# huangjh-pub/di-fusion

Hardware: AMD Instinct MI355X
Metric: frames/s integrate+decode+mesh, 640x480 synthetic stream (higher is better)
Workload: dtype f32

## Files before the change

di_fusion_amd/csrc/kernels_extract.hip.h:

```cpp
#pragma once

__device__ __forceinline__ void mark_confident_nbhd(const Geo& g, int lin, float ignore_th, const int64_t* __restrict__ indexer,
                                                    const float* __restrict__ obs, const GridMarks& marks) {
    const uint32_t* bits = marks.bits;
    int ix, iy, iz;
    unlinearize(g, lin, ix, iy, iz);
    int cand[7];
    cand[0] = lin;
    cand[1] = linearize(g, clampi(ix - 1, 0, g.nx - 1), iy, iz);
    cand[2] = linearize(g, clampi(ix + 1, 0, g.nx - 1), iy, iz);
    cand[3] = linearize(g, ix, clampi(iy - 1, 0, g.ny - 1), iz);
    cand[4] = linearize(g, ix, clampi(iy + 1, 0, g.ny - 1), iz);
    cand[5] = linearize(g, ix, iy, clampi(iz - 1, 0, g.nz - 1));
    cand[6] = linearize(g, ix, iy, clampi(iz + 1, 0, g.nz - 1));
    int64_t slot[7];
#pragma unroll
    for (int c = 0; c < 7; ++c) slot[c] = indexer[cand[c]];
    float w[7];
#pragma unroll
    for (int c = 0; c < 7; ++c) w[c] = slot[c] >= 0 ? obs[slot[c]] : ignore_th;
    uint32_t word[7];
#pragma unroll
    for (int c = 0; c < 7; ++c) word[c] = (w[c] > ignore_th) ? bits[cand[c] >> 5] : 0xFFFFFFFFu;
    uint32_t prev[7];
#pragma unroll
    for (int c = 0; c < 7; ++c) {
        const uint32_t b = 1u << (cand[c] & 31);
        prev[c] = (word[c] & b) ? 0xFFFFFFFFu : atomicOr(marks.bits + (cand[c] >> 5), b);
    }
#pragma unroll
    for (int c = 0; c < 7; ++c)
        if (!(prev[c] & (1u << (cand[c] & 31)))) atomicAdd(marks.tot + (cand[c] >> 5) / marks.per_words, 1);
}

__global__ void __launch_bounds__(DIF_BLOCK) k_mark_halo_dirty(Geo g, float ignore_th, uint8_t* __restrict__ dirty, const int64_t* __restrict__ pos,
                                                             const int64_t* __restrict__ indexer, const float* __restrict__ obs,
                                                             GridMarks bits, const int* __restrict__ n_ptr, int64_t own_lo,
                                                             int64_t own_hi) {
    const int n = *n_ptr;
    for (int s = blockIdx.x * blockDim.x + threadIdx.x; s < n; s += gridDim.x * blockDim.x) {
        if (!dirty[s]) continue;
        const int64_t p = pos[s];
        if (p >= own_lo && p < own_hi) continue;
        dirty[s] = 0;
        mark_confident_nbhd(g, (int)p, ignore_th, indexer, obs, bits);
    }
}

struct DirtySet {
    uint8_t* dirty;
    const int64_t* pos;
    int64_t* valid_blocks;
    int* counters;
    int no_cache;
    int64_t max_voxels;
    Geo g;
    float ignore_th;
    const int64_t* indexer;
    const float* obs;
    GridMarks bits;
    int64_t own_lin_lo, own_lin_hi;
    bool tiled;
    __device__ __forceinline__ bool owned(int s) const {
        if (!tiled) return true;
        const int64_t p = pos[s];
        return p >= own_lin_lo && p < own_lin_hi;
    }
};

struct DirtyFunctor {
    DirtySet a;
    __device__ int count(int s) const { return ((a.no_cache || a.dirty[s]) && a.owned(s)) ? 1 : 0; }
    __device__ void emit(int s, int offset) const {
        a.dirty[s] = 0;
        if (offset >= a.max_voxels) return;
        const int lin = (int)a.pos[s];
        a.valid_blocks[offset] = lin;
        mark_confident_nbhd(a.g, lin, a.ignore_th, a.indexer, a.obs, a.bits);
    }
    __device__ void finish(int total) const {
        if (total > a.max_voxels) { total = (int)a.max_voxels; a.counters[DIF_C_OVERFLOW] = 2; }
        a.counters[DIF_C_K] = total;
        a.counters[DIF_C_DEFERRED] = 0;
    }
};

__device__ __forceinline__ void dirty_scan_body(const DirtySet& a, const int* __restrict__ n_ptr, const int* __restrict__ block_tot,
                                                uint32_t* __restrict__ fused_word, int seq) {
    __shared__ int smem[8];
    if (fused_word && blockIdx.x == 0 && threadIdx.x == 0) __hip_atomic_store(fused_word, (uint32_t)seq, __ATOMIC_RELAXED, __HIP_MEMORY_SCOPE_AGENT);
    const int s = (int)blockIdx.x * DIF_BLOCK + (int)threadIdx.x;
    const bool flag = a.dirty[s] != 0;
    if (!__syncthreads_or((int)flag) && blockIdx.x != 0) return;
    int before = 0, all = 0;
    const int n_blk = (int)gridDim.x;
    for (int b = (int)threadIdx.x; b < n_blk; b += DIF_BLOCK) {
        const int t = block_tot[b];
        all += t;
        if (b < (int)blockIdx.x) before += t;
    }
    const GridMarks& marks = a.bits;
    int lin = 0, cand[7];
    uint32_t word[7];
#pragma unroll
    for (int c = 0; c < 7; ++c) { cand[c] = 0; word[c] = 0xFFFFFFFFu; }
    if (flag && (lin = (int)a.pos[s]) >= 0) {
        int ix, iy, iz;
        unlinearize(a.g, lin, ix, iy, iz);
        cand[0] = lin;
        cand[1] = linearize(a.g, clampi(ix - 1, 0, a.g.nx - 1), iy, iz);
        cand[2] = linearize(a.g, clampi(ix + 1, 0, a.g.nx - 1), iy, iz);
        cand[3] = linearize(a.g, ix, clampi(iy - 1, 0, a.g.ny - 1), iz);
        cand[4] = linearize(a.g, ix, clampi(iy + 1, 0, a.g.ny - 1), iz);
        cand[5] = linearize(a.g, ix, iy, clampi(iz - 1, 0, a.g.nz - 1));
        cand[6] = linearize(a.g, ix, iy, clampi(iz + 1, 0, a.g.nz - 1));
        int64_t slot[7];
#pragma unroll
        for (int c = 0; c < 7; ++c) slot[c] = a.indexer[cand[c]];
        float w[7];
#pragma unroll
        for (int c = 0; c < 7; ++c) w[c] = slot[c] >= 0 ? a.obs[slot[c]] : a.ignore_th;
#pragma unroll
        for (int c = 0; c < 7; ++c) word[c] = (w[c] > a.ignore_th) ? marks.bits[cand[c] >> 5] : 0xFFFFFFFFu;
    }
    const int n = *n_ptr;
    const bool mine = flag && s < n;
    int offset = block_sum(before, smem);
    const int total = block_sum(all, smem);
    {
        const int64_t need = min((int64_t)7 * total, (int64_t)n);
        if (need > a.max_voxels) {
            if (blockIdx.x == 0 && threadIdx.x == 0) { a.counters[DIF_C_K] = 0; a.counters[DIF_C_DEFERRED] = (int)need; }
            return;
        }
    }
    int chunk_total;
    const int ex = block_excl_scan(mine ? 1 : 0, smem, chunk_total);
    if (mine) {
        a.dirty[s] = 0;
        if (offset + ex < a.max_voxels) {
            a.valid_blocks[offset + ex] = lin;
            uint32_t prev[7];
#pragma unroll
            for (int c = 0; c < 7; ++c) {
                const uint32_t b = 1u << (cand[c] & 31);
                prev[c] = (word[c] & b) ? 0xFFFFFFFFu : atomicOr(marks.bits + (cand[c] >> 5), b);
            }
#pragma unroll
            for (int c = 0; c < 7; ++c)
                if (!(prev[c] & (1u << (cand[c] & 31)))) atomicAdd(marks.tot + (cand[c] >> 5) / marks.per_words, 1);
        }
    }
    if (blockIdx.x == 0 && threadIdx.x == 0) {
        int t = total;
        if (t > a.max_voxels) { t = (int)a.max_voxels; a.counters[DIF_C_OVERFLOW] = 2; }
        a.counters[DIF_C_K] = t;
        a.counters[DIF_C_DEFERRED] = 0;
    }
}

__global__ void __launch_bounds__(DIF_BLOCK) k_dirty_scan(DirtySet a, const int* __restrict__ n_ptr, const int* __restrict__ block_tot, uint32_t* __restrict__ fused_word, int seq) {
    dirty_scan_body(a, n_ptr, block_tot, fused_word, seq);
}
struct DirtyScanArgs { DirtySet a; const int* n_ptr; const int* block_tot; };
__global__ void __launch_bounds__(DIF_BLOCK) k_dirty_scan_batch(Batch<DirtyScanArgs> b) {
    const DirtyScanArgs& a = b.s[blockIdx.y];
    dirty_scan_body(a.a, a.n_ptr, a.block_tot, nullptr, 0);
}
__global__ void k_publish_word(uint32_t* __restrict__ word, uint32_t value) {
    if (threadIdx.x == 0) __hip_atomic_store(word, value, __ATOMIC_RELAXED, __HIP_MEMORY_SCOPE_AGENT);
}

struct OccFunctor {
    uint32_t* bits;
    const int64_t* indexer;
    int32_t* occ_slot;
    int32_t* vbm;
    int* counters;
    int64_t max_voxels;
    __device__ int count(int w) const { return __popc(bits[w]); }
    __device__ void emit(int w, int offset) const {
        uint32_t word = bits[w];
        bits[w] = 0u;
        while (word) {
            int b = __ffs((int)word) - 1;
            word &= word - 1;
            int slot = (int)indexer[w * 32 + b];
            if (offset < max_voxels) {
                occ_slot[offset] = slot;
                vbm[slot] = offset;
            }
            ++offset;
        }
    }
    __device__ void finish(int total) const {
        if (total > max_voxels) { total = (int)max_voxels; counters[DIF_C_OVERFLOW] = 3; }
        counters[DIF_C_B] = total;
        counters[DIF_C_VH] = 0;
        counters[DIF_C_WORK] = 0;
    }
};

struct Lattice {
    int res;
    float vsize, a;
    __device__ __forceinline__ float coord(int i) const { return ((float)i * vsize + a) - 0.5f; }
};

struct DecodeArgs {
    int mode;
    const int* n_ptr;
    int64_t n_static;
    Lattice lat;
    const int32_t* occ_slot;
    const float* latent;
    const int32_t* list;
    const float* rows;
    const float* xyz;
    const int64_t* indexer;
    Geo geo;
    float* out_sdf;
    float* out_std;
    float sign;
    float* out_grad;
    const float* wbwd;
    float grad_scale;
    const float* fold_table;
    const float* obs;
    float ignore_th;
    float pose[12];
    int* zero_word;
};

__device__ __forceinline__ float pose_row(const float* T, int j, float x, float y, float z) {
    return __fadd_rn(__fadd_rn(__fadd_rn(__fmul_rn(x, T[4 * j]), __fmul_rn(y, T[4 * j + 1])), __fmul_rn(z, T[4 * j + 2])), T[4 * j + 3]);
}

struct DecodeRow { bool live; int64_t out_idx; float px, py, pz; bool bad; };
template <bool DENSE = false>
__device__ __forceinline__ DecodeRow decode_row_input(const DecodeArgs& A, int64_t tile, int col, int half, int res3, int tiles_per_voxel, int64_t n_rows,
                                                      f16v& xin) {
    DecodeRow R{false, 0, 0.f, 0.f, 0.f, false};
    const float* lat_row = nullptr;
    const float* row32 = nullptr;
    if (!DENSE && A.mode == 0) {
        const int64_t b = tile / tiles_per_voxel;
        const int s = (int)(tile - b * tiles_per_voxel) * 32 + col;
        R.live = s < res3;
        if (R.live) {
            const int r = A.lat.res;
            R.px = A.lat.coord(s / (r * r)); R.py = A.lat.coord((s / r) % r); R.pz = A.lat.coord(s % r);
            lat_row = A.latent + (int64_t)A.occ_slot[b] * L;
            R.out_idx = b * res3 + s;
        }
    } else if (!DENSE && A.mode == 1) {
        const int64_t row = tile * 32 + col;
        R.live = row < n_rows;
        if (R.live) {
            const int e = A.list[row];
            const int b = e / res3, s = e - b * res3, r = A.lat.res;
            R.px = A.lat.coord(s / (r * r)); R.py = A.lat.coord((s / r) % r); R.pz = A.lat.coord(s % r);
            lat_row = A.latent + (int64_t)A.occ_slot[b] * L;
            R.out_idx = e;
        }
    } else if (!DENSE && A.mode == 2) {
        const int64_t row = tile * 32 + col;
        R.live = row < n_rows;
        if (R.live) { row32 = A.rows + row * 32; R.out_idx = row; }
    } else if (DENSE) {
        const int64_t row = tile * 32 + col;
        if (row < n_rows) {
            const float x = A.xyz[row * 3 + 0], y = A.xyz[row * 3 + 1], z = A.xyz[row * 3 + 2];
            float xn, yn, zn; int ix, iy, iz;
            bool ok = voxel_of(A.geo, pose_row(A.pose, 0, x, y, z), pose_row(A.pose, 1, x, y, z), pose_row(A.pose, 2, x, y, z), xn, yn, zn, ix, iy, iz);
            int64_t slot = -1;
            if (ok) {
                slot = A.indexer[linearize(A.geo, ix, iy, iz)];
                ok = slot >= 0 && A.obs[slot] > A.ignore_th;
            }
            R.live = ok;
            R.out_idx = row;
            if (ok) {
                R.px = (xn - (float)ix) - 0.5f; R.py = (yn - (float)iy) - 0.5f; R.pz = (zn - (float)iz) - 0.5f;
                lat_row = A.latent + slot * L;
            } else if (half == 1) A.out_std[row] = 0.0f;
        }
    } else {
        const int64_t row = tile * 32 + col;
        R.live = row < n_rows;
        if (R.live) {
            const int64_t p = A.list[row];
            float xn, yn, zn; int ix, iy, iz;
            voxel_of(A.geo, A.xyz[p * 3 + 0], A.xyz[p * 3 + 1], A.xyz[p * 3 + 2], xn, yn, zn, ix, iy, iz);
            R.px = (xn - (float)ix) - 0.5f; R.py = (yn - (float)iy) - 0.5f; R.pz = (zn - (float)iz) - 0.5f;
            lat_row = A.latent + A.indexer[linearize(A.geo, ix, iy, iz)] * L;
            R.out_idx = row;
        }
    }
#pragma unroll
    for (int t = 0; t < 16; ++t) {
        const int k = 2 * t + half;
        float v = 0.0f;
        if (R.live) {
            if (row32) v = row32[k];
            else if (k < L) v = lat_row[k];
            else v = (k == L) ? R.px : ((k == L + 1) ? R.py : R.pz);
        }
        xin[t] = v;
    }
    if constexpr (!DENSE) {
        if (A.mode == 2) {
            unsigned nf = 0;
#pragma unroll
            for (int t = 0; t < 16; ++t) nf |= ((__float_as_uint(xin[t]) & 0x7f800000u) == 0x7f800000u) ? 1u : 0u;
            nf |= (unsigned)__shfl_xor((int)nf, 32);
            R.bad = nf != 0;
        }
    }
    return R;
}

template <bool GRAD, bool DENSE = false>
__global__ void __launch_bounds__(GRAD ? 256 : 512, GRAD ? 1 : 2) k_decode(DecodeArgs A, const float* __restrict__ wblob) {
    extern __shared__ __attribute__((aligned(16))) float lds[];
    if (DENSE && A.zero_word && blockIdx.x == 0 && threadIdx.x == 0) *A.zero_word = 0;
    stage_weights(lds, wblob, DEC_LDS_FLOATS);
    const __amdgpu_buffer_rsrc_t wfwd = make_rsrc(wblob, DEC_FLOATS);
    const __amdgpu_buffer_rsrc_t wbwd = make_rsrc(GRAD ? A.wbwd : wblob, GRAD ? DECB_FLOATS : DEC_FLOATS);
    const int lane = lane_id(), half = lane >> 5, col = lane & 31;
    const int wave = (int)((threadIdx.x >> 6) * gridDim.x + blockIdx.x);
    const int nwaves = (int)(gridDim.x * (blockDim.x >> 6));
    const int res3 = A.lat.res * A.lat.res * A.lat.res;
    const int tiles_per_voxel = (res3 + 31) / 32;
    int64_t n_rows, n_tiles;
    if (A.mode == 0) {
        n_rows = (int64_t)(*A.n_ptr) * res3;
        n_tiles = (int64_t)(*A.n_ptr) * tiles_per_voxel;
    } else {
        n_rows = A.n_ptr ? (int64_t)(*A.n_ptr) : A.n_static;
        n_tiles = (n_rows + 31) / 32;
    }
    for (int64_t tile = wave; tile < n_tiles; tile += nwaves) {
        f16v xin;
        const DecodeRow R = decode_row_input<DENSE>(A, tile, col, half, res3, tiles_per_voxel, n_rows, xin);
        const bool live = R.live;
        const int64_t out_idx = R.out_idx;
        const float px = R.px, py = R.py, pz = R.pz;
        float sdf, sd;
        if (!GRAD && A.mode == 1 && A.fold_table) {
            const int b = live ? A.list[tile * 32 + col] / res3 : 0;
            decoder_tile_folded(lds, wfwd, FoldInitGlobal{A.fold_table + (int64_t)b * 256}, px, py, pz, lane, sdf, sd);
        } else if (GRAD) {
            float gx, gy, gz;
            decoder_tile_grad(lds, wfwd, wbwd, xin, lane, sdf, sd, gx, gy, gz);
            if (live && half == 1) {
                const float gs = R.bad ? __builtin_nanf("") : A.grad_scale;
                A.out_grad[out_idx * 3 + 0] = gx * gs;
                A.out_grad[out_idx * 3 + 1] = gy * gs;
                A.out_grad[out_idx * 3 + 2] = gz * gs;
            }
        } else {
            decoder_tile(lds, wfwd, xin, lane, sdf, sd);
        }
        if (live) {
            if (half == 0) A.out_sdf[out_idx] = R.bad ? __builtin_nanf("") : A.sign * sdf;
            else A.out_std[out_idx] = R.bad ? __builtin_nanf("") : sd;
        }
    }
}

template <bool DENSE = false>
__global__ void __launch_bounds__(512, 1) k_decode_x6(DecodeArgs A, const float* __restrict__ wblob, const float* __restrict__ wu) {
    extern __shared__ __attribute__((aligned(16))) float lds[];
    if (DENSE && A.zero_word && blockIdx.x == 0 && threadIdx.x == 0) *A.zero_word = 0;
    stage_weights(lds, wblob, X6_LDS_BYTES / 4);
    const __amdgpu_buffer_rsrc_t wfwd = make_rsrc(wblob, X6_BYTES / 4);
    const __amdgpu_buffer_rsrc_t wun = make_rsrc(wu, X6U_BYTES / 4);
    const int lane = lane_id(), half = lane >> 5, col = lane & 31;
    const int wave = (int)((threadIdx.x >> 6) * gridDim.x + blockIdx.x);
    const int nwaves = (int)(gridDim.x * (blockDim.x >> 6));
    const int res3 = A.lat.res * A.lat.res * A.lat.res;
    const int tiles_per_voxel = (res3 + 31) / 32;
    int64_t n_rows, n_tiles;
    if (A.mode == 0) {
        n_rows = (int64_t)(*A.n_ptr) * res3;
        n_tiles = (int64_t)(*A.n_ptr) * tiles_per_voxel;
    } else {
        n_rows = A.n_ptr ? (int64_t)(*A.n_ptr) : A.n_static;
        n_tiles = (n_rows + 31) / 32;
    }
    for (int64_t tile = wave; tile < n_tiles; tile += nwaves) {
        f16v xin;
        const DecodeRow R = decode_row_input<DENSE>(A, tile, col, half, res3, tiles_per_voxel, n_rows, xin);
        const bool live = R.live;
        const int64_t out_idx = R.out_idx;
        float sdf, sd;
        decoder_tile_x6(lds, wfwd, wun, xin, lane, sdf, sd);
        if (live) {
            if (half == 0) A.out_sdf[out_idx] = R.bad ? __builtin_nanf("") : A.sign * sdf;
            else A.out_std[out_idx] = R.bad ? __builtin_nanf("") : sd;
        }
    }
}

#ifndef GRAD_X6_THREADS
#define GRAD_X6_THREADS 256
#endif
template <int PF, bool DENSE = false>
__global__ void __launch_bounds__(GRAD_X6_THREADS, 1) k_decode_grad_x6(DecodeArgs A, const float* __restrict__ wblob, const float* __restrict__ wu,
                                                          const float* __restrict__ wb) {
    extern __shared__ __attribute__((aligned(16))) float lds[];
    if (DENSE && A.zero_word && blockIdx.x == 0 && threadIdx.x == 0) *A.zero_word = 0;
    stage_weights(lds, wblob, X6_LDS_BYTES / 4);
    const __amdgpu_buffer_rsrc_t wfwd = make_rsrc(wblob, X6_BYTES / 4);
    const __amdgpu_buffer_rsrc_t wun = make_rsrc(wu, X6U_BYTES / 4);
    const __amdgpu_buffer_rsrc_t wbw = make_rsrc(wb, X6B_BYTES / 4);
    const int lane = lane_id(), half = lane >> 5, col = lane & 31;
    const int wave = (int)((threadIdx.x >> 6) * gridDim.x + blockIdx.x);
    const int nwaves = (int)(gridDim.x * (blockDim.x >> 6));
    const int res3 = A.lat.res * A.lat.res * A.lat.res;
    const int64_t n_rows = A.n_ptr ? (int64_t)(*A.n_ptr) : A.n_static;
    const int64_t n_tiles = (n_rows + 31) / 32;
    for (int64_t tile = wave; tile < n_tiles; tile += nwaves) {
        f16v xin;
        const DecodeRow R = decode_row_input<DENSE>(A, tile, col, half, res3, 1, n_rows, xin);
        float sdf, sd, gx, gy, gz;
        decoder_tile_grad_x6<PF>(lds, wfwd, wun, wbw, xin, lane, sdf, sd, gx, gy, gz);
        if (R.live) {
            if (half == 0) A.out_sdf[R.out_idx] = R.bad ? __builtin_nanf("") : A.sign * sdf;
            else {
                const float gs = R.bad ? __builtin_nanf("") : A.grad_scale;
                A.out_std[R.out_idx] = R.bad ? __builtin_nanf("") : sd;
                A.out_grad[R.out_idx * 3 + 0] = gx * gs;
                A.out_grad[R.out_idx * 3 + 1] = gy * gs;
                A.out_grad[R.out_idx * 3 + 2] = gz * gs;
            }
        }
    }
}

template <int NS>
__device__ __forceinline__ void decode_refine_x6_body(const BatchN<DecodeArgs, NS>& B, int S, const float* __restrict__ wblob) {
    extern __shared__ __attribute__((aligned(16))) float lds[];
    const int lane = lane_id(), half = lane >> 5, col = lane & 31;
    const int wave = __builtin_amdgcn_readfirstlane((int)((threadIdx.x >> 6) * gridDim.x + blockIdx.x));
    const int nwaves = (int)(gridDim.x * (blockDim.x >> 6));
    const Lattice lat = B.s[0].lat;
    const float sign = B.s[0].sign;
    const int res3 = lat.res * lat.res * lat.res, r = lat.res;
    Ranges<NS, int64_t> rg;
    rg.pre[0] = 0;
#pragma unroll
    for (int j = 0; j < NS; ++j) {
        rg.cnt[j] = (j < S) ? (B.s[j].n_ptr ? (int64_t)(*B.s[j].n_ptr) : B.s[j].n_static) : 0;
        rg.pre[j + 1] = rg.pre[j] + (rg.cnt[j] + 31) / 32;
    }
    const int64_t n_tiles = rg.total();
    int sm_n; int64_t lt_n, rows_n;
    rg.locate(wave, sm_n, lt_n, rows_n);
    int e_next = (wave < n_tiles && lt_n * 32 + col < rows_n) ? B.s[sm_n].list[lt_n * 32 + col] : 0;
    __builtin_amdgcn_sched_barrier(0);
    stage_weights(lds, wblob, X6_LDS_BYTES / 4);
    const __amdgpu_buffer_rsrc_t wfwd = make_rsrc(wblob, X6_BYTES / 4);
    for (int64_t T = wave; T < n_tiles; T += nwaves) {
        const int sm = sm_n;
        const int64_t tile = lt_n, n_rows = rows_n;
        const DecodeArgs& A = B.s[sm];
        const int64_t row = tile * 32 + col;
        const bool live = row < n_rows;
        const int e = e_next;
        rg.locate(T + nwaves, sm_n, lt_n, rows_n);
        e_next = (T + nwaves < n_tiles && lt_n * 32 + col < rows_n) ? B.s[sm_n].list[lt_n * 32 + col] : 0;
        const int b = e / res3, sb = e - b * res3;
        const float px = lat.coord(sb / (r * r)), py = lat.coord((sb / r) % r), pz = lat.coord(sb % r);
        float sdf, sd;
        decoder_tile_folded_x6(lds, wfwd, FoldInitGlobal{A.fold_table + (int64_t)b * 256}, px, py, pz, lane, sdf, sd);
        if (live) {
            if (half == 0) A.out_sdf[e] = sign * sdf;
            else A.out_std[e] = sd;
        }
    }
}

__global__ void __launch_bounds__(512, 1) k_decode_refine_x6(DecodeArgs A, const float* __restrict__ wblob) {
    const BatchN<DecodeArgs, 1> B{{A}};
    decode_refine_x6_body<1>(B, 1, wblob);
}
__global__ void __launch_bounds__(512, 1) k_decode_refine_x6_batch(Batch<DecodeArgs> B, int S, const float* __restrict__ wblob) {
    decode_refine_x6_body<DIF_MAX_STREAMS>(B, S, wblob);
}

__device__ __forceinline__ void tri_axis(int j, int l, float scale, int& i0, int& i1, float& w0, float& w1) {
    float src = scale * (float)j;
    i0 = min((int)src, l - 1);
    i1 = i0 + ((i0 < l - 1) ? 1 : 0);
    w1 = fminf(fmaxf(src - (float)i0, 0.0f), 1.0f);
    w0 = 1.0f - w1;
}

__device__ __forceinline__ float tri_sample(const float* __restrict__ low, int l, int x0, int x1, int y0, int y1, int z0, int z1,
                                            float wx0, float wx1, float wy0, float wy1, float wz0, float wz1) {
    float v00 = fmaf(low[(x0 * l + y0) * l + z0], wz0, low[(x0 * l + y0) * l + z1] * wz1);
    float v01 = fmaf(low[(x0 * l + y1) * l + z0], wz0, low[(x0 * l + y1) * l + z1] * wz1);
    float v10 = fmaf(low[(x1 * l + y0) * l + z0], wz0, low[(x1 * l + y0) * l + z1] * wz1);
    float v11 = fmaf(low[(x1 * l + y1) * l + z0], wz0, low[(x1 * l + y1) * l + z1] * wz1);
    float v0 = fmaf(v00, wy0, v01 * wy1);
    float v1 = fmaf(v10, wy0, v11 * wy1);
    return fmaf(v0, wx0, v1 * wx1);
}

__global__ void __launch_bounds__(DIF_BLOCK) k_upsample_mark(const float* __restrict__ low_sdf, const float* __restrict__ low_std, int l, int R,
                                                           float* __restrict__ cube_sdf, float* __restrict__ cube_std,
                                                           int32_t* __restrict__ refine_list, int* __restrict__ counters) {
    __shared__ int smem[8];
    __shared__ int s_base;
    const int B = counters[DIF_C_B];
    const int R2 = R * R, R3 = R2 * R, l3 = l * l * l;
    const int64_t n_rows = (int64_t)B * R2;
    const float scale = (float)(l - 1) / (float)(R - 1);
    const int64_t stride = (int64_t)gridDim.x * blockDim.x;
    const int64_t n_pad = (n_rows + DIF_BLOCK - 1) / DIF_BLOCK * DIF_BLOCK;
    for (int64_t row = (int64_t)blockIdx.x * blockDim.x + threadIdx.x; row < n_pad; row += stride) {
        unsigned sel = 0;
        int64_t e0 = 0;
        if (row < n_rows) {
            const int b = (int)(row / R2), jxy = (int)(row - (int64_t)b * R2);
            const int jx = jxy / R, jy = jxy % R;
            int x0, x1, y0, y1; float wx0, wx1, wy0, wy1;
            tri_axis(jx, l, scale, x0, x1, wx0, wx1);
            tri_axis(jy, l, scale, y0, y1, wy0, wy1);
            const float* ls = low_sdf + (int64_t)b * l3;
            const float* ld = low_std + (int64_t)b * l3;
            e0 = (int64_t)b * R3 + (int64_t)jxy * R;
            NO_PACKED_F32
            for (int jz = 0; jz < R; ++jz) {
                int z0, z1; float wz0, wz1;
                tri_axis(jz, l, scale, z0, z1, wz0, wz1);
                float sv = tri_sample(ls, l, x0, x1, y0, y1, z0, z1, wx0, wx1, wy0, wy1, wz0, wz1);
                float dv = tri_sample(ld, l, x0, x1, y0, y1, z0, z1, wx0, wx1, wy0, wy1, wz0, wz1);
                cube_sdf[e0 + jz] = -sv;
                cube_std[e0 + jz] = dv;
                if (fabsf(sv) < 0.05f) sel |= 1u << jz;
            }
        }
        int total;
        int ex = block_excl_scan(__popc(sel), smem, total);
        if (total > 0) {
            if (threadIdx.x == 0) s_base = atomicAdd(counters + DIF_C_VH, total);
            __syncthreads();
            int o = s_base + ex;
            while (sel) {
                int jz = __ffs((int)sel) - 1;
                sel &= sel - 1;
                refine_list[o++] = (int32_t)(e0 + jz);
            }
        }
        __syncthreads();
    }
}

struct VoxelDecodeArgs {
    const int32_t* occ_slot;
    const float* latent;
    Lattice low;
    int R;
    float* cube_sdf;
    float* cube_std;
    int32_t* refine_list;
    int* counters;
    const float* fold_w;
    float* fold_table;
};

#define VD_MAX_L3 64
#define VD_MAX_R2 64
#define VD_WAVE_LDS_FLOATS (2 * VD_MAX_L3 + 2 * 256)

#ifdef DIF_TRACE
__device__ unsigned long long g_vd_trace[2048 * 8];
#define VD_STAMP(slot) do { if (lane_id() == 0) g_vd_trace[((threadIdx.x >> 6) * gridDim.x + blockIdx.x) * 8 + (slot)] = wall_clock64(); } while (0)
#else
#define VD_STAMP(slot) do { } while (0)
#endif

template <bool X6, int NS>
__device__ __forceinline__ void decode_voxels_body(const BatchN<VoxelDecodeArgs, NS>& AB, int S, const float* __restrict__ wblob) {
    extern __shared__ __attribute__((aligned(16))) float lds[];
    VD_STAMP(0);
    constexpr int LDS_W = X6 ? X6_LDS_BYTES / 4 : ((DEC_LDS_FLOATS + 3) & ~3);
#if defined(DIF_VD_CUT) && DIF_VD_CUT == 0
    return;
#endif
    stage_weights(lds, wblob, X6 ? X6_LDS_BYTES / 4 : DEC_LDS_FLOATS);
    VD_STAMP(1);
#if defined(DIF_VD_CUT) && DIF_VD_CUT == 1
    return;
#endif
    const __amdgpu_buffer_rsrc_t wfwd = make_rsrc(wblob, X6 ? X6_BYTES / 4 : DEC_FLOATS);
    const int lane = lane_id(), half = lane >> 5, col = lane & 31, wid = threadIdx.x >> 6;
    const int pair = wid >> 1, tsel = wid & 1;
    float* w_low_sdf = lds + LDS_W + pair * VD_WAVE_LDS_FLOATS;
    float* w_low_std = w_low_sdf + VD_MAX_L3;
    float* w_fold = w_low_std + VD_MAX_L3 + tsel * 256;
    const Lattice low = AB.s[0].low;
    const float* const fold_w = AB.s[0].fold_w;
    const int l = low.res, R = AB.s[0].R, l3 = l * l * l, R2 = R * R, R3 = R2 * R;
    const float scale = (float)(l - 1) / (float)(R - 1);
    int pre[NS + 1];
    pre[0] = 0;
#pragma unroll
    for (int j = 0; j < NS; ++j) pre[j + 1] = pre[j] + ((j < S) ? AB.s[j].counters[DIF_C_B] : 0);
    const int B = pre[NS];
    const int pairs_per_block = (int)(blockDim.x >> 7), n_pairs = (int)gridDim.x * pairs_per_block;
    const int first = __builtin_amdgcn_readfirstlane(pair * (int)gridDim.x + (int)blockIdx.x);
    __shared__ int s_tot[8], s_map[8], s_base[NS];
    const int rounds = (B + n_pairs - 1) / n_pairs;
    for (int round = 0; round < rounds; ++round) {
        const int bg = first + round * n_pairs;
        int sm = 0, b = bg;
#pragma unroll
        for (int j = 1; j < NS; ++j)
            if (bg >= pre[j]) { sm = j; b = bg - pre[j]; }
        const VoxelDecodeArgs& A = AB.s[sm];
        unsigned sel = 0;
        const int jz0 = tsel * (R >> 1), jz1 = jz0 + (R >> 1);
        const int64_t e0 = (int64_t)b * R3 + (int64_t)lane * R;
        if (bg < B && tsel * 32 < l3) {
            const float* lat_row = A.latent + (int64_t)A.occ_slot[b] * L;
            const int s = tsel * 32 + col;
            const float px = low.coord(s / (l * l)), py = low.coord((s / l) % l), pz = low.coord(s % l);
            float sdf = 0.0f, sd = 0.0f;
            if (X6 || fold_w) {
                if constexpr (X6) decoder_fold_consts_x6(lds, fold_w, lat_row, w_fold, lane);
                else decoder_fold_consts(lds, fold_w, lat_row, w_fold, lane);
                __builtin_amdgcn_wave_barrier();
                __builtin_amdgcn_s_waitcnt(0xc07f);
                if (tsel == 0) {
                    float* rec = A.fold_table + (int64_t)b * 256;
                    for (int p = lane; p < 256; p += 64) rec[p] = w_fold[p];
                }
                VD_STAMP(6);
#if defined(DIF_VD_CUT) && DIF_VD_CUT == 2
                sdf = w_fold[lane]; sd = w_fold[lane + 64];
#else
                if constexpr (X6) decoder_tile_folded_x6(lds, wfwd, FoldInitLds{w_fold}, px, py, pz, lane, sdf, sd);
                else decoder_tile_folded(lds, wfwd, FoldInitLds{w_fold}, px, py, pz, lane, sdf, sd);
#endif
            } else if constexpr (!X6) {
                f16v xin;
#pragma unroll
                for (int t = 0; t < 16; ++t) {
                    const int k = 2 * t + half;
                    xin[t] = (k < L) ? lat_row[k] : 0.0f;
                }
                if (half) { xin[14] = px; xin[15] = pz; } else { xin[15] = py; }
                decoder_tile(lds, wfwd, xin, lane, sdf, sd);
            }
            if (s < l3) {
                if (half == 0) w_low_sdf[s] = sdf;
                else w_low_std[s] = sd;
            }
        }
        __syncthreads();
        VD_STAMP(2);
        if (bg < B && lane < R2) {
            const int jx = lane / R, jy = lane % R;
            int x0, x1, y0, y1; float wx0, wx1, wy0, wy1;
            tri_axis(jx, l, scale, x0, x1, wx0, wx1);
            tri_axis(jy, l, scale, y0, y1, wy0, wy1);
            float* const cube_sdf = A.cube_sdf;
            float* const cube_std = A.cube_std;
            for (int jz = jz0; jz < jz1; ++jz) {
                int z0, z1; float wz0, wz1;
                tri_axis(jz, l, scale, z0, z1, wz0, wz1);
                float sv = tri_sample(w_low_sdf, l, x0, x1, y0, y1, z0, z1, wx0, wx1, wy0, wy1, wz0, wz1);
                float dv = tri_sample(w_low_std, l, x0, x1, y0, y1, z0, z1, wx0, wx1, wy0, wy1, wz0, wz1);
                cube_sdf[e0 + jz] = -sv;
                cube_std[e0 + jz] = dv;
                if (fabsf(sv) < 0.05f) sel |= 1u << jz;
            }
        }
        VD_STAMP(3);
        const int c = __popc(sel);
        const int incl = wave_incl_scan(c);
        const int total = __shfl(incl, 63);
        if (lane == 0) { s_tot[wid] = total; if (NS > 1) s_map[wid] = sm; }
        __syncthreads();
        if (NS == 1) {
            if (threadIdx.x == 0) {
                int sum = 0;
                for (int w = 0; w < (int)(blockDim.x >> 6); ++w) sum += s_tot[w];
                s_base[0] = sum ? atomicAdd(A.counters + DIF_C_VH, sum) : 0;
            }
        } else if ((int)threadIdx.x < S) {
            const int j = (int)threadIdx.x;
            int sum = 0;
            for (int w = 0; w < (int)(blockDim.x >> 6); ++w) sum += (s_map[w] == j) ? s_tot[w] : 0;
            s_base[j] = sum ? atomicAdd(AB.s[j].counters + DIF_C_VH, sum) : 0;
        }
        __syncthreads();
        if (total > 0) {
            int o = s_base[NS == 1 ? 0 : sm] + incl - c;
            for (int w = 0; w < wid; ++w) o += (NS == 1 || s_map[w] == sm) ? s_tot[w] : 0;
            int32_t* const refine_list = A.refine_list;
            while (sel) {
                const int jz = __ffs((int)sel) - 1;
                sel &= sel - 1;
                refine_list[o++] = (int32_t)(e0 + jz);
            }
        }
        __syncthreads();
        VD_STAMP(4);
    }
    VD_STAMP(5);
}

template <bool X6>
__global__ void __launch_bounds__(512, X6 ? 1 : 2) k_decode_voxels(VoxelDecodeArgs A, const float* __restrict__ wblob) {
    const BatchN<VoxelDecodeArgs, 1> B{{A}};
    decode_voxels_body<X6, 1>(B, 1, wblob);
}
template <bool X6>
__global__ void __launch_bounds__(512, X6 ? 1 : 2) k_decode_voxels_batch(Batch<VoxelDecodeArgs> B, int S, const float* __restrict__ wblob) {
    decode_voxels_body<X6, DIF_MAX_STREAMS>(B, S, wblob);
}
```

Measured before the change: 10030.

## Software-pipeline voxel decode across two wave cohorts to overlap decode and upsample

Adds a pipelined path for the X6 decoder, used when there are more voxel batches than wave pairs. Waves are split into two cohorts that alternate by step. While one cohort runs the MLP decoder tile, the other upsamples the previous batch, writes refine-list entries, reserves atomic offsets and precomputes fold constants for the next batch. The goal is to hide decoder compute behind memory-bound upsampling and to cut the number of block-wide syncs and atomics per batch. The cost is more complex shared-state handoff through s_tot/s_off, which raises the risk of synchronisation bugs.

Result: slower. 9740 (-2.9%).

```diff
diff --git a/di_fusion_amd/csrc/kernels_extract.hip.h b/di_fusion_amd/csrc/kernels_extract.hip.h
--- a/di_fusion_amd/csrc/kernels_extract.hip.h
+++ b/di_fusion_amd/csrc/kernels_extract.hip.h
@@ -583,6 +583,131 @@
 #define VD_STAMP(slot) do { } while (0)
 #endif
 
+__device__ __forceinline__ unsigned vd_upsample_row(const float* low_sdf, const float* low_std, int l, int R, float scale, int lane, int jz0, int jz1,
+                                                    float* cube_sdf, float* cube_std, int64_t e0) {
+    const int jx = lane / R, jy = lane % R;
+    int x0, x1, y0, y1; float wx0, wx1, wy0, wy1;
+    tri_axis(jx, l, scale, x0, x1, wx0, wx1);
+    tri_axis(jy, l, scale, y0, y1, wy0, wy1);
+    unsigned sel = 0;
+    for (int jz = jz0; jz < jz1; ++jz) {
+        int z0, z1; float wz0, wz1;
+        tri_axis(jz, l, scale, z0, z1, wz0, wz1);
+        float sv = tri_sample(low_sdf, l, x0, x1, y0, y1, z0, z1, wx0, wx1, wy0, wy1, wz0, wz1);
+        float dv = tri_sample(low_std, l, x0, x1, y0, y1, z0, z1, wx0, wx1, wy0, wy1, wz0, wz1);
+        cube_sdf[e0 + jz] = -sv;
+        cube_std[e0 + jz] = dv;
+        if (fabsf(sv) < 0.05f) sel |= 1u << jz;
+    }
+    return sel;
+}
+
+template <int NS>
+__device__ __forceinline__ void decode_voxels_pipelined(const BatchN<VoxelDecodeArgs, NS>& AB, int S, const int (&pre)[NS + 1], float* __restrict__ lds,
+                                                        const __amdgpu_buffer_rsrc_t wfwd, float* __restrict__ w_low_sdf, float* __restrict__ w_low_std,
+                                                        float* __restrict__ w_fold) {
+    const int lane = lane_id(), col = lane & 31, half = lane >> 5;
+    const int wid = __builtin_amdgcn_readfirstlane((int)(threadIdx.x >> 6));
+    const int tsel = wid & 1, cohort = wid >> 2;
+    const Lattice low = AB.s[0].low;
+    const float* const fold_w = AB.s[0].fold_w;
+    const int l = low.res, R = AB.s[0].R, l3 = l * l * l, R2 = R * R, R3 = R2 * R;
+    const float scale = (float)(l - 1) / (float)(R - 1);
+    const int B = pre[NS];
+    const int H = 2 * (int)gridDim.x;
+    const int first = __builtin_amdgcn_readfirstlane(((wid >> 1) & 1) * (int)gridDim.x + (int)blockIdx.x);
+    const int nh = (B + H - 1) / H;
+    const int jz0 = tsel * (R >> 1), jz1 = jz0 + (R >> 1);
+    const bool has_tile = tsel * 32 < l3;
+    const bool leader = (wid & 3) == 0;
+    const int w_other = 4 * (1 - cohort);
+    __shared__ int s_tot[8], s_map[8], s_off[8];
+    auto locate = [&](int bg, int& sm, int& b) {
+        sm = 0; b = bg;
+#pragma unroll
+        for (int j = 1; j < NS; ++j)
+            if (bg >= pre[j]) { sm = j; b = bg - pre[j]; }
+    };
+    unsigned sel_c = 0;
+    int bg_c = 0;
+    for (int t = -1; t < nh + 3; ++t) {
+        if ((t & 1) == cohort) {
+            const int bg = t * H + first;
+            if (t >= 0 && t < nh && bg < B && has_tile) {
+                const int s = tsel * 32 + col;
+                const float px = low.coord(s / (l * l)), py = low.coord((s / l) % l), pz = low.coord(s % l);
+                float sdf = 0.0f, sd = 0.0f;
+                decoder_tile_folded_x6(lds, wfwd, FoldInitLds{w_fold}, px, py, pz, lane, sdf, sd);
+                if (s < l3) {
+                    if (half == 0) w_low_sdf[s] = sdf;
+                    else w_low_std[s] = sd;
+                }
+            }
+        } else {
+            const bool reserve = leader && t - 2 >= 0 && t - 2 < nh && lane < (NS == 1 ? 1 : S);
+            int base = 0;
+            if (reserve) {
+                int sum = 0;
+                for (int w = w_other; w < w_other + 4; ++w) sum += (NS == 1 || s_map[w] == lane) ? s_tot[w] : 0;
+                if (sum) base = atomicAdd(AB.s[NS == 1 ? 0 : lane].counters + DIF_C_VH, sum);
+            }
+            unsigned sel = 0;
+            const int bg_u = (t - 1) * H + first;
+            const bool posted = t - 1 >= 0 && t - 1 < nh;
+            int sm_u = 0;
+            if (posted && bg_u < B) {
+                int b;
+                locate(bg_u, sm_u, b);
+                const VoxelDecodeArgs& A = AB.s[sm_u];
+                if (lane < R2) sel = vd_upsample_row(w_low_sdf, w_low_std, l, R, scale, lane, jz0, jz1, A.cube_sdf, A.cube_std, (int64_t)b * R3 + (int64_t)lane * R);
+            }
+            {
+                const int c = __popc(sel_c);
+                const int incl = wave_incl_scan(c);
+                if (__shfl(incl, 63) > 0) {
+                    int sm, b;
+                    locate(bg_c, sm, b);
+                    const int64_t e0 = (int64_t)b * R3 + (int64_t)lane * R;
+                    int32_t* const refine_list = AB.s[sm].refine_list;
+                    int o = s_off[wid] + incl - c;
+                    while (sel_c) {
+                        const int jz = __ffs((int)sel_c) - 1;
+                        sel_c &= sel_c - 1;
+                        refine_list[o++] = (int32_t)(e0 + jz);
+                    }
+                }
+            }
+            if (posted) {
+                int total = __popc(sel);
+#pragma unroll
+                for (int d = 32; d >= 1; d >>= 1) total += __shfl_xor(total, d);
+                if (lane == 0) { s_tot[wid] = total; if (NS > 1) s_map[wid] = sm_u; }
+            }
+            sel_c = sel;
+            bg_c = bg_u;
+            const int bg_f = (t + 1) * H + first;
+            if (t + 1 < nh && bg_f < B && has_tile) {
+                int sm, b;
+                locate(bg_f, sm, b);
+                const VoxelDecodeArgs& A = AB.s[sm];
+                decoder_fold_consts_x6(lds, fold_w, A.latent + (int64_t)A.occ_slot[b] * L, w_fold, lane);
+                __builtin_amdgcn_wave_barrier();
+                __builtin_amdgcn_s_waitcnt(0xc07f);
+                if (tsel == 0) {
+                    float* rec = A.fold_table + (int64_t)b * 256;
+                    for (int p = lane; p < 256; p += 64) rec[p] = w_fold[p];
+                }
+            }
+            if (reserve) {
+                int o = base;
+                for (int w = w_other; w < w_other + 4; ++w)
+                    if (NS == 1 || s_map[w] == lane) { s_off[w] = o; o += s_tot[w]; }
+            }
+        }
+        __syncthreads();
+    }
+}
+
 template <bool X6, int NS>
 __device__ __forceinline__ void decode_voxels_body(const BatchN<VoxelDecodeArgs, NS>& AB, int S, const float* __restrict__ wblob) {
     extern __shared__ __attribute__((aligned(16))) float lds[];
@@ -614,6 +739,13 @@
     const int pairs_per_block = (int)(blockDim.x >> 7), n_pairs = (int)gridDim.x * pairs_per_block;
     const int first = __builtin_amdgcn_readfirstlane(pair * (int)gridDim.x + (int)blockIdx.x);
     __shared__ int s_tot[8], s_map[8], s_base[NS];
+    if constexpr (X6) {
+        if (B > n_pairs) {
+            decode_voxels_pipelined<NS>(AB, S, pre, lds, wfwd, w_low_sdf, w_low_std, w_fold);
+            VD_STAMP(5);
+            return;
+        }
+    }
     const int rounds = (B + n_pairs - 1) / n_pairs;
     for (int round = 0; round < rounds; ++round) {
         const int bg = first + round * n_pairs;
@@ -663,23 +795,7 @@
         }
         __syncthreads();
         VD_STAMP(2);
-        if (bg < B && lane < R2) {
-            const int jx = lane / R, jy = lane % R;
-            int x0, x1, y0, y1; float wx0, wx1, wy0, wy1;
-            tri_axis(jx, l, scale, x0, x1, wx0, wx1);
-            tri_axis(jy, l, scale, y0, y1, wy0, wy1);
-            float* const cube_sdf = A.cube_sdf;
-            float* const cube_std = A.cube_std;
-            for (int jz = jz0; jz < jz1; ++jz) {
-                int z0, z1; float wz0, wz1;
-                tri_axis(jz, l, scale, z0, z1, wz0, wz1);
-                float sv = tri_sample(w_low_sdf, l, x0, x1, y0, y1, z0, z1, wx0, wx1, wy0, wy1, wz0, wz1);
-                float dv = tri_sample(w_low_std, l, x0, x1, y0, y1, z0, z1, wx0, wx1, wy0, wy1, wz0, wz1);
-                cube_sdf[e0 + jz] = -sv;
-                cube_std[e0 + jz] = dv;
-                if (fabsf(sv) < 0.05f) sel |= 1u << jz;
-            }
-        }
+        if (bg < B && lane < R2) sel = vd_upsample_row(w_low_sdf, w_low_std, l, R, scale, lane, jz0, jz1, A.cube_sdf, A.cube_std, e0);
         VD_STAMP(3);
         const int c = __popc(sel);
         const int incl = wave_incl_scan(c);
```
